# t0037799/INT8InferenceEngine

Measured on AMD Instinct MI355X. Metric: images/sec AlexNet-INT8 224x224 bs=1000, higher is better.
Workload: dtype int8; 1 GPU; alexnet INT8 forward + top-1, 3x224x224 input, global batch 1000 sharded over 1 GPU(s); global_batch=1000, per_gpu_batch=1000, parallelism=batch-shard x1 + logits all-gather

## Files before the change

int8inferenceengine_amd/csrc/i8ie_stem.hip:

```cpp
#include <cstdio>
#include <cstdlib>
#include <type_traits>
#include <vector>

#include "i8ie_stem.h"
#include "i8ie_stem_common.h"

#if !defined(STEM_DMA_VEC)
#define STEM_DMA_VEC 0
#endif

#if defined(STEM_PRIO_SWAP)
#define STEM_VPRIO 0
#define STEM_MPRIO 3
#endif

namespace {

__device__ __forceinline__ uint32_t quant_exact(float x, float scale, float zpf, float rscale) {
  const float est = __builtin_fmaf(x, rscale, zpf);
  const float fr = __builtin_amdgcn_fractf(est);
  if (__builtin_fabsf(est) < 1024.0f && __builtin_fabsf(fr - 0.5f) <= 0.5f - 9.765625e-4f)
    return (uint32_t)((int)est) & 0xFFu;
  const float t = x / scale + zpf;
  return (uint32_t)((int)t) & 0xFFu;
}

template <bool F32>
__global__ __launch_bounds__(256) void quantize_s2d_kernel(const void* __restrict__ xin, uint8_t* __restrict__ out, uint32_t total,
                                                           int c, int h, int w, int HY, int WX, int pad, float scale, float zpf,
                                                           float rscale, uint32_t zp) {
  const uint32_t gstride = gridDim.x * 256u;
  const size_t cs = (size_t)h * w;
  for (uint32_t e = blockIdx.x * 256u + threadIdx.x; e < total; e += gstride) {
    const uint32_t d = e & 3u, t0 = e >> 2;
    const uint32_t t1 = t0 / (uint32_t)WX, X = t0 - t1 * WX;
    const uint32_t img = t1 / (uint32_t)HY, Y = t1 - img * HY;
    const int y = (int)(4 * Y + d) - pad, x0 = (int)(4 * X) - pad;
    const bool yin = y >= 0 && y < h;
    const int yc = y < 0 ? 0 : (y >= h ? h - 1 : y);
    uint32_t q[12];
    if constexpr (F32) {
      const float* plane = static_cast<const float*>(xin) + ((size_t)img * c * h + yc) * w;
      const bool vec = (w & 1) == 0 && (pad & 1) == 0 && w >= 4 && (reinterpret_cast<uintptr_t>(xin) & 7u) == 0;
      const int xb = x0 < 0 ? 0 : (x0 > w - 4 ? w - 4 : x0);
      const int sft = x0 - xb;
#pragma unroll
      for (int ch = 0; ch < 3; ++ch) {
        const float* row = plane + (size_t)(ch < c ? ch : 0) * cs;
        float L[4];
        if (vec) {
          const float2 a = *reinterpret_cast<const float2*>(row + xb), b = *reinterpret_cast<const float2*>(row + xb + 2);
          L[0] = a.x; L[1] = a.y; L[2] = b.x; L[3] = b.y;
        } else {
#pragma unroll
          for (int i = 0; i < 4; ++i) {
            const int xx = xb + i;
            L[i] = row[xx < 0 ? 0 : (xx >= w ? w - 1 : xx)];
          }
        }
#pragma unroll
        for (int px = 0; px < 4; ++px) {
          int i = px + sft;
          i = i < 0 ? 0 : (i > 3 ? 3 : i);
          const float v = i == 0 ? L[0] : (i == 1 ? L[1] : (i == 2 ? L[2] : L[3]));
          q[px * 3 + ch] = quant_exact(v, scale, zpf, rscale);
        }
      }
    } else {
      const uint8_t* plane = static_cast<const uint8_t*>(xin) + ((size_t)img * c * h + yc) * w;
#pragma unroll
      for (int ch = 0; ch < 3; ++ch) {
        const uint8_t* row = plane + (size_t)(ch < c ? ch : 0) * cs;
#pragma unroll
        for (int px = 0; px < 4; ++px) {
          const int xx = x0 + px;
          q[px * 3 + ch] = row[xx < 0 ? 0 : (xx >= w ? w - 1 : xx)];
        }
      }
    }
    uint32_t wd[3] = {0, 0, 0};
#pragma unroll
    for (int px = 0; px < 4; ++px) {
      const int xx = x0 + px;
      const bool in = yin && xx >= 0 && xx < w;
#pragma unroll
      for (int ch = 0; ch < 3; ++ch) {
        const uint32_t v = (in && ch < c) ? q[px * 3 + ch] : zp;
        const int b = px * 3 + ch;
        wd[b >> 2] |= v << (8 * (b & 3));
      }
    }
    uint32_t* o = reinterpret_cast<uint32_t*>(out) + (size_t)e * 3;
    o[0] = wd[0] ^ 0x80808080u;
    o[1] = wd[1] ^ 0x80808080u;
    o[2] = wd[2] ^ 0x80808080u;
  }
}

template <int NG, int KS, bool ACC, bool PC>
__global__ __launch_bounds__(512, 2) void stem_conv_kernel(StemArgs p) {
  uint8_t* const smem = stem_smem;
  const int tid = threadIdx.x, lane = tid & 63;
  const int wave_hw = __builtin_amdgcn_readfirstlane(tid >> 6);
  const int wave = p.role_split ? ((wave_hw & 2) << 1) | ((wave_hw >> 2) << 1) | (wave_hw & 1) : wave_hw;
  const int hh = lane >> 5, l31 = lane & 31;

  const int n_units = p.n_img << p.lg_parts;
  const int n_mine = ((int)blockIdx.x < n_units) ? (n_units - 1 - (int)blockIdx.x) / (int)gridDim.x + 1 : 0;
  if (n_mine == 0) return;
  const int T = p.T, G = n_mine * T, RING = p.RING;
  const int pmask = p.parts - 1;

  for (int i = tid; i < p.N; i += 512) reinterpret_cast<int*>(smem + p.lds_ocp)[i] = p.ocp[i];
  for (int i = tid; i < KS * 64; i += 512) {
    const int j = i >> 6, ln = i & 63;
    *reinterpret_cast<v4i*>(smem + p.lds_bfrag + i * 16) =
        *reinterpret_cast<const v4i*>(p.B + (size_t)((NG - 1) * 32 + (ln & 31)) * p.Kpad + j * 32 + (ln >> 5) * 16);
  }
  stem_fill_tables(p, smem, tid, T, RING);
  __syncthreads();
  auto strip_fetch = [&](int unit, int t, v4i& a, v4i& b) {
    const int idx = (unit & pmask) * T + t;
    a = *reinterpret_cast<const v4i*>(smem + p.lds_tab + idx * 32);
    b = *reinterpret_cast<const v4i*>(smem + p.lds_tab + idx * 32 + 16);
  };
  auto strip_decode = [&](const v4i& a, const v4i& b) {
    StemStrip e;
    e.lo = __builtin_amdgcn_readfirstlane(a.x); e.hi = __builtin_amdgcn_readfirstlane(a.y);
    e.poff = __builtin_amdgcn_readfirstlane(a.z); e.pbytes = __builtin_amdgcn_readfirstlane(a.w);
    e.j0 = __builtin_amdgcn_readfirstlane(b.x); e.j1 = __builtin_amdgcn_readfirstlane(b.y);
    e.lom = __builtin_amdgcn_readfirstlane(b.z); e.jm = __builtin_amdgcn_readfirstlane(b.w);
    return e;
  };
  auto strip = [&](int unit, int t) {
    v4i a, b;
    strip_fetch(unit, t, a, b);
    return strip_decode(a, b);
  };
  auto adv_of = [&](int unit) { return __builtin_amdgcn_readfirstlane(reinterpret_cast<const int*>(smem + p.lds_adv)[unit & pmask]); };
  auto patch_dma = [&](int unit, const StemStrip& e, int pb) {
    if (e.pbytes <= 0) return;
    const __amdgpu_buffer_rsrc_t rs = __builtin_amdgcn_make_buffer_rsrc(
        const_cast<uint8_t*>(p.img + (size_t)(unit >> p.lg_parts) * p.img_pitch + (unsigned)e.poff), 0, e.pbytes, 0x00020000);
    const int pieces = (e.pbytes + 1023) >> 10;
    uint8_t* dst = smem + p.lds_patch + pb * p.patchB;
    for (int q = wave & 3; q < pieces; q += 4)
      __builtin_amdgcn_raw_ptr_buffer_load_lds(rs, (__attribute__((address_space(3))) void*)(dst + q * 1024), 16, (q * 64 + lane) * 16, 0, 0, 0);
  };

  if (wave < 4) {
#if defined(STEM_MPRIO)
    __builtin_amdgcn_s_setprio(STEM_MPRIO);
#endif
    constexpr int NA = NG - 1;
    v4i breg[NA > 0 ? NA : 1][KS];
#pragma unroll
    for (int g = 0; g < NA; ++g) {
      const int8_t* brow = p.B + (size_t)(g * 32 + l31) * p.Kpad + hh * 16;
#pragma unroll
      for (int j = 0; j < KS; ++j) breg[g][j] = *reinterpret_cast<const v4i*>(brow + j * 32);
    }
    int koff[KS];
    {
      int q = hh, run = 0, rem = hh;
#pragma unroll
      for (int j = 0; j < KS; ++j) {
        koff[j] = q < p.nch ? run * p.rowB + rem * 16 : 0;
        q += 2;
        rem += 2;
        while (rem >= p.RC) {
          rem -= p.RC;
          ++run;
        }
      }
    }
    const int pp = wave * 32 + l31;
    int lr = (int)((float)pp * p.rcpOW), lx = pp - lr * p.OW;
    if (lx < 0) { lx += p.OW; --lr; } else if (lx >= p.OW) { lx -= p.OW; ++lr; }
    const int aoff = (lr * p.sq * p.WX + lx * p.sq) * 48;
    const int roff = lx * p.pitchP + 16 * hh;
    int t = 0, un = (int)blockIdx.x, ib = 0, pbuf = 0;
    int tn = 0, imn = (int)blockIdx.x;
    auto next_n = [&]() {
      if (++tn == T) {
        tn = 0;
        imn += (int)gridDim.x;
      }
    };
    StemStrip e = strip(imn, tn);
    patch_dma(imn, e, 0);
    next_n();
    v4i fa, fb;
    strip_fetch(imn, tn, fa, fb);
    asm volatile("s_waitcnt vmcnt(0)" ::: "memory");
    STEM_BAR();
    for (int g = 0; g < G; ++g) {
      StemStrip en{};
      if (g + 1 < G) {
        en = strip_decode(fa, fb);
        if (!STEM_DMA_VEC) patch_dma(imn, en, pbuf ^ 1);
        next_n();
      }
      const int npx = (e.hi - e.lo) * p.OW;
      if (wave * 32 < npx) {
        const bool valid = pp < npx;
        const uint8_t* abase = smem + p.lds_patch + pbuf * p.patchB + (valid ? aoff : 0);
        int slot = ib + e.lom;
        if (slot >= RING) slot -= RING;
        int ls = slot + lr;
        if (ls >= RING) ls -= RING;
        uint8_t* const rbase = smem + p.lds_ring + ls * p.ringRowB + roff;
        v16i acc[NG];
        const v16i z = {0, 0, 0, 0, 0, 0, 0, 0, 0, 0, 0, 0, 0, 0, 0, 0};
        uint8_t* const wbase = valid ? rbase : smem + p.lds_dump + lane * 16;
        auto ring_store = [&](auto ggc, auto qc) {
          constexpr int gg = decltype(ggc)::value, q = decltype(qc)::value;
          v4i v;
          v.x = acc[gg][q * 4 + 0]; v.y = acc[gg][q * 4 + 1]; v.z = acc[gg][q * 4 + 2]; v.w = acc[gg][q * 4 + 3];
          *reinterpret_cast<v4i*>(wbase + (gg * 32 + 8 * q) * 4) = v;
        };
        {
          constexpr int DB = KS < 4 ? KS : 4;
          v4i ring[DB], bring[DB];
          const uint8_t* const bbase = smem + p.lds_bfrag + lane * 16;
          static_for<0, DB>([&](auto jc) {
            constexpr int j = decltype(jc)::value;
            ring[j] = *reinterpret_cast<const v4i*>(abase + koff[j]);
            bring[j] = *reinterpret_cast<const v4i*>(bbase + j * 1024);
          });
          __builtin_amdgcn_sched_barrier(0);
          static_for<0, KS>([&](auto jc) {
            constexpr int j = decltype(jc)::value;
            const v4i af = ring[j % DB], bf = bring[j % DB];
            if constexpr (j + DB < KS) {
              ring[j % DB] = *reinterpret_cast<const v4i*>(abase + koff[j + DB]);
              bring[j % DB] = *reinterpret_cast<const v4i*>(bbase + (j + DB) * 1024);
              __builtin_amdgcn_sched_barrier(0);
            }
#pragma unroll
            for (int gg = 0; gg < NA; ++gg) acc[gg] = __builtin_amdgcn_mfma_i32_32x32x32_i8(breg[gg][j], af, j == 0 ? z : acc[gg], 0, 0, 0);
            acc[NG - 1] = __builtin_amdgcn_mfma_i32_32x32x32_i8(bf, af, j == 0 ? z : acc[NG - 1], 0, 0, 0);
            __builtin_amdgcn_sched_barrier(0);
          });
          if constexpr (NA > 0)
            static_for<0, 4 * NA>([&](auto ic) { ring_store(std::integral_constant<int, decltype(ic)::value / 4>{}, std::integral_constant<int, decltype(ic)::value % 4>{}); });
        }
        static_for<0, 4>([&](auto qc) { ring_store(std::integral_constant<int, NG - 1>{}, qc); });
      }
      strip_fetch(imn, tn, fa, fb);
      if (!STEM_DMA_VEC) asm volatile("s_waitcnt vmcnt(0)" ::: "memory");
      STEM_BAR();
      if (++t == T) {
        t = 0;
        ib += adv_of(un);
        if (ib >= RING) ib -= RING;
        un += (int)gridDim.x;
      }
      pbuf ^= 1;
      e = en;
    }
    STEM_BAR();
    return;
  }

  const int vt = (wave - 4) * 64 + lane;
  const int vwave = wave - 4;
#if !defined(STEM_VPRIO)
#define STEM_VPRIO 0
#endif
  if (STEM_VPRIO) __builtin_amdgcn_s_setprio(STEM_VPRIO);
  const I8ieRequant rq = p.rq;
  const int lo_relu = p.relu_lo;
  const float lof = (float)lo_relu;
  const int N4 = p.N >> 2;
  const int PHp = p.PH + 2 * p.ob, PWp = p.PW + 2 * p.ob;
  const __amdgpu_buffer_rsrc_t rsO =
      __builtin_amdgcn_make_buffer_rsrc(p.out, 0, p.out_bytes, 0x00020000);
  const int hg = ((l31 >= 4 && l31 < 12) || (l31 >= 16 && l31 < 20) || l31 >= 28) ? 1 : 0;
  const int gi = hg == 0 ? (l31 < 4 ? l31 : (l31 < 16 ? l31 - 8 : l31 - 12)) : (l31 < 12 ? l31 - 4 : (l31 < 20 ? l31 - 8 : l31 - 16));
  const int pl = gi & 7;
  const int ql = 2 * (2 * hh + hg) + (gi >> 3);
  const int nqo = N4 >> 3, npo = (p.PW + 7) >> 3, ntask = nqo * npo;
  constexpr int PITCH = NG * 128 + 16;
  const int rd_lane = pl * p.ps * PITCH + ql * 16;
  const int st_lane = pl * p.N + ql * 4;

  constexpr int UN = 3;
  struct PoolTask {
    int rd, st, oc;
  };
  auto task_of = [&](int k) {
    int po = k < ntask ? k : 0, qo = 0;
    while (po >= npo) {
      po -= npo;
      ++qo;
    }
    const bool ok = 8 * po + pl < p.PW;
    PoolTask t;
    t.rd = (ok ? rd_lane : ql * 16) + (8 * po) * p.ps * PITCH + qo * 128;
    t.st = ok && k < ntask ? (8 * po) * p.N + qo * 32 + st_lane : (int)0x80000000;
    t.oc = p.lds_ocp + (qo * 8 + ql) * 16;
    return t;
  };
  PoolTask tk0[UN];
#pragma unroll
  for (int u = 0; u < UN; ++u) tk0[u] = task_of(vwave + 4 * u);
  v4i oc0[UN];
#pragma unroll
  for (int u = 0; u < UN; ++u) oc0[u] = *reinterpret_cast<const v4i*>(smem + tk0[u].oc);
  int nst = 0;
  auto pool_rows = [&](auto pkc, int im, int ib, const StemStrip& e) {
    constexpr int PK = decltype(pkc)::value;
    int rm = ib + e.jm;
    if (rm >= RING) rm -= RING;
    for (int j = e.j0; j < e.j1; ++j) {
      int rowoff[PK];
#pragma unroll
      for (int dy = 0; dy < PK; ++dy) {
        const int sl = rm + dy;
        rowoff[dy] = p.lds_ring + (sl >= RING ? sl - RING : sl) * p.ringRowB;
      }
      const int orow = ((im * PHp + j + p.ob) * PWp + p.ob) * p.N;
      auto round = [&](const PoolTask (&tk)[UN], const v4i (&ocv)[UN]) {
        float4 msq[UN];
        if constexpr (PC) {
#pragma unroll
          for (int u = 0; u < UN; ++u) msq[u] = *reinterpret_cast<const float4*>(p.msv + ((tk[u].oc - p.lds_ocp) >> 2));
        }
        v4i v[UN][PK * PK];
#pragma unroll
        for (int u = 0; u < UN; ++u)
#pragma unroll
          for (int dy = 0; dy < PK; ++dy) {
            const uint8_t* const a = smem + (rowoff[dy] + tk[u].rd);
#pragma unroll
            for (int dx = 0; dx < PK; ++dx) v[u][dy * PK + dx] = *reinterpret_cast<const v4i*>(a + dx * PITCH);
          }
        uint32_t d[UN];
        float worst[UN];
        int c4[UN][4];
#pragma unroll
        for (int u = 0; u < UN; ++u) {
          v4i m = v[u][0];
#pragma unroll
          for (int tt = 1; tt < PK * PK; ++tt) {
            m.x = m.x > v[u][tt].x ? m.x : v[u][tt].x;
            m.y = m.y > v[u][tt].y ? m.y : v[u][tt].y;
            m.z = m.z > v[u][tt].z ? m.z : v[u][tt].z;
            m.w = m.w > v[u][tt].w ? m.w : v[u][tt].w;
          }
          c4[u][0] = m.x + ocv[u].x; c4[u][1] = m.y + ocv[u].y;
          c4[u][2] = m.z + ocv[u].z; c4[u][3] = m.w + ocv[u].w;
          if constexpr (PC) d[u] = i8ie_requant_est4_pc(c4[u], rq, msq[u], lof, worst[u]);
          else d[u] = i8ie_requant_est4(c4[u], rq, lof, worst[u]);
        }
        float wmin = worst[0];
#pragma unroll
        for (int u = 1; u < UN; ++u) wmin = __builtin_fminf(wmin, worst[u]);
        if (!i8ie_requant_est_ok(wmin)) {
#pragma unroll
          for (int u = 0; u < UN; ++u)
            if (!i8ie_requant_est_ok(worst[u])) {
              if constexpr (PC) d[u] = i8ie_requant_exact4_pc(c4[u], rq, p.sbv + ((tk[u].oc - p.lds_ocp) >> 2), lo_relu);
              else d[u] = i8ie_requant_exact4(c4[u], rq, lo_relu);
            }
        }
#pragma unroll
        for (int u = 0; u < UN; ++u) __builtin_amdgcn_raw_buffer_store_b32(d[u] ^ p.xor_out, rsO, tk[u].st, orow, 0);
        nst += UN;
      };
      round(tk0, oc0);
      for (int k0 = vwave + 4 * UN; k0 < ntask; k0 += 4 * UN) {
        PoolTask tk[UN];
        v4i ocv[UN];
#pragma unroll
        for (int u = 0; u < UN; ++u) {
          tk[u] = task_of(k0 + 4 * u);
          ocv[u] = *reinterpret_cast<const v4i*>(smem + tk[u].oc);
        }
        round(tk, ocv);
      }
      rm += p.ps;
      if (rm >= RING) rm -= RING;
    }
  };
  auto dump_acc = [&](int im, int ib, const StemStrip& e) {
    const int tasks = (e.hi - e.lo) * p.OW * N4;
    const float rn4 = 1.0f / (float)N4;
    for (int id = vt; id < tasks; id += 256) {
      int t1 = (int)((float)id * rn4), qq = id - t1 * N4;
      if (qq < 0) { qq += N4; --t1; } else if (qq >= N4) { qq -= N4; ++t1; }
      int r = 0, x = t1;
      while (x >= p.OW) {
        x -= p.OW;
        ++r;
      }
      int sl = ib + e.lom + r;
      while (sl >= RING) sl -= RING;
      const v4i v = *reinterpret_cast<const v4i*>(smem + p.lds_ring + sl * p.ringRowB + x * p.pitchP + qq * 16);
      const v4i o = *reinterpret_cast<const v4i*>(smem + p.lds_ocp + qq * 16);
      const int4 c = make_int4(v.x + o.x, v.y + o.y, v.z + o.z, v.w + o.w);
      *reinterpret_cast<int4*>(p.acc + ((size_t)im * (size_t)(p.OH * p.OW) + (size_t)((e.lo + r) * p.OW + x)) * (size_t)p.N + qq * 4) = c;
    }
  };
  auto wait_vm_keep = [&](int keep) {
    switch (keep < 16 ? keep : 16) {
      case 0: asm volatile("s_waitcnt vmcnt(0)" ::: "memory"); break;
      case 1: asm volatile("s_waitcnt vmcnt(1)" ::: "memory"); break;
      case 2: asm volatile("s_waitcnt vmcnt(2)" ::: "memory"); break;
      case 3: asm volatile("s_waitcnt vmcnt(3)" ::: "memory"); break;
      case 4: asm volatile("s_waitcnt vmcnt(4)" ::: "memory"); break;
      case 5: asm volatile("s_waitcnt vmcnt(5)" ::: "memory"); break;
      case 6: asm volatile("s_waitcnt vmcnt(6)" ::: "memory"); break;
      case 7: asm volatile("s_waitcnt vmcnt(7)" ::: "memory"); break;
      case 8: asm volatile("s_waitcnt vmcnt(8)" ::: "memory"); break;
      case 9: asm volatile("s_waitcnt vmcnt(9)" ::: "memory"); break;
      case 10: asm volatile("s_waitcnt vmcnt(10)" ::: "memory"); break;
      case 11: asm volatile("s_waitcnt vmcnt(11)" ::: "memory"); break;
      case 12: asm volatile("s_waitcnt vmcnt(12)" ::: "memory"); break;
      case 13: asm volatile("s_waitcnt vmcnt(13)" ::: "memory"); break;
      case 14: asm volatile("s_waitcnt vmcnt(14)" ::: "memory"); break;
      case 15: asm volatile("s_waitcnt vmcnt(15)" ::: "memory"); break;
      default: asm volatile("s_waitcnt vmcnt(16)" ::: "memory"); break;
    }
  };

  int t1 = 0, im1 = (int)blockIdx.x, ib1 = 0;
  int tn = 1, imn = (int)blockIdx.x;
  if (tn == T) {
    tn = 0;
    imn += (int)gridDim.x;
  }
  v4i fa, fb;
  strip_fetch(im1, t1, fa, fb);
  STEM_BAR();
  for (int g = 0; g <= G; ++g) {
    if (STEM_DMA_VEC && g + 1 < G) {
      patch_dma(imn, strip(imn, tn), (g + 1) & 1);
      if (++tn == T) {
        tn = 0;
        imn += (int)gridDim.x;
      }
      nst = 0;
    }
    if (g >= 1) {
      const StemStrip e = strip_decode(fa, fb);
      const int img = im1 >> p.lg_parts;
      if (e.j1 > e.j0) {
        if (p.pk == 3) pool_rows(std::integral_constant<int, 3>{}, img, ib1, e);
        else if (p.pk == 2) pool_rows(std::integral_constant<int, 2>{}, img, ib1, e);
        else pool_rows(std::integral_constant<int, 1>{}, img, ib1, e);
      }
      if constexpr (ACC) {
        if (e.hi > e.lo) dump_acc(img, ib1, e);
      }
      if (++t1 == T) {
        t1 = 0;
        ib1 += adv_of(im1);
        if (ib1 >= RING) ib1 -= RING;
        im1 += (int)gridDim.x;
      }
    }
    strip_fetch(im1, t1, fa, fb);
    if constexpr (ACC) wait_vm_keep(0);
    else if (STEM_DMA_VEC) wait_vm_keep(nst);
    STEM_BAR();
  }
}

template <int NG, int KS, bool ACC, bool PC>
int launch_stem_t(i8ie_ctx* ctx, const StemArgs& a, int grid, int lds) {
  static bool raised[64] = {};
  const int dev = ctx->device & 63;
  if (!raised[dev]) {
    I8IE_HIP_TRY(hipFuncSetAttribute(reinterpret_cast<const void*>(&stem_conv_kernel<NG, KS, ACC, PC>), hipFuncAttributeMaxDynamicSharedMemorySize, 160 * 1024));
    raised[dev] = true;
  }
  stem_conv_kernel<NG, KS, ACC, PC><<<grid, 512, lds, ctx->stream>>>(a);
  I8IE_LAUNCH_CHECK();
  return I8IE_OK;
}
template <int NG, int KS>
int launch_stem(i8ie_ctx* ctx, const StemArgs& a, int grid, int lds) {
  if (a.msv != nullptr)
    return a.acc != nullptr ? launch_stem_t<NG, KS, true, true>(ctx, a, grid, lds) : launch_stem_t<NG, KS, false, true>(ctx, a, grid, lds);
  return a.acc != nullptr ? launch_stem_t<NG, KS, true, false>(ctx, a, grid, lds) : launch_stem_t<NG, KS, false, false>(ctx, a, grid, lds);
}

struct StemPlan {
  int KC4, KA4, HY, WX, K2, KS, KST, NR, first, T, parts, pk, ps, PH, PW, carry, RING, pitchP, ringRowB, patchB, lds_tab, lds_adv, lds_dump, lds_bfrag, lds;
};

bool stem_plan(int c, int stride, int N, int KH, int KW, int OH, int OW, int pool_k, int pool_s, int parts, StemPlan* out) {
  if (c > 3 || c < 1 || stride < 4 || stride % 4 != 0) return false;
  if (N % 32 != 0 || N < 32 || N > 96) return false;
  if (pool_k == 1 && pool_s > 1) return false;
  StemPlan s{};
  const int sq = stride / 4;
  s.KC4 = (KH + 3) / 4;
  s.KA4 = (KW + 3) / 4;
  s.HY = (OH - 1) * sq + s.KC4;
  s.WX = (OW - 1) * sq + s.KA4;
  s.K2 = s.KC4 * s.KA4 * 48;
  s.KS = (s.K2 + 31) / 32;
  if (s.KS > kStemMaxKS || s.KS < 2) return false;
  s.pk = pool_k > 1 ? pool_k : 1;
  s.ps = pool_k > 1 ? pool_s : 1;
  if (s.ps < 1 || s.ps > s.pk || s.pk > 3) return false;
  if (s.pk > OH || s.pk > OW) return false;
  s.PH = (OH - s.pk) / s.ps + 1;
  s.PW = (OW - s.pk) / s.ps + 1;
  s.carry = s.pk - s.ps;
  int NR = kStemPix / OW;
  NR -= NR % s.ps;
  if (NR < 1 || NR < s.carry) return false;
  if (NR > 8) NR = 8 - 8 % s.ps;
  s.NR = NR;
  s.first = s.carry > 0 ? s.carry : NR;
  if (s.first > OH) s.first = OH;
  if (parts != 1 && parts != 2 && parts != 4) return false;
  if (s.PH < 2 * parts) return false;
  s.parts = parts;
  auto J0_of = [&](int q) { return q * s.PH / parts; };
  auto R0_of = [&](int q) { return J0_of(q) * s.ps; };
  auto R1_of = [&](int q) { return q + 1 == parts ? OH : (J0_of(q + 1) - 1) * s.ps + s.pk; };
  s.T = 1;
  for (int q = 0; q < parts; ++q) {
    const int rows = R1_of(q) - R0_of(q);
    const int t = 1 + (rows > s.first ? (rows - s.first + NR - 1) / NR : 0);
    if (t > s.T) s.T = t;
  }
  s.RING = 2 * NR + s.carry;
  s.pitchP = N * 4 + 16;
  s.ringRowB = OW * s.pitchP;
  const int prmax = (NR - 1) * sq + s.KC4;
  s.patchB = ((prmax * s.WX * 48 + 1023) & ~1023) + 1024;
  if (s.T * parts > 256) return false;
  s.KST = s.KS <= 6 ? 6 : (s.KS <= 10 ? 10 : kStemMaxKS);
  s.lds_tab = 2 * s.patchB + s.RING * s.ringRowB + N * 4 + 64;
  s.lds_adv = s.lds_tab + s.T * parts * 32;
  s.lds_dump = s.lds_adv + 16;
  s.lds_bfrag = s.lds_dump + 2048;
  s.lds = s.lds_bfrag + s.KST * 1024;
  if (s.lds > 160 * 1024) return false;
  for (int qa = 0; qa < parts; ++qa)
    for (int qb = 0; qb < parts; ++qb) {
      const int q_of[2] = {qa, qb};
      const int base[2] = {0, R1_of(qa) - R0_of(qa)};
      auto hi_of = [&](int u, int t) { const int v = R0_of(q_of[u]) + s.first + t * s.NR; return v < R1_of(q_of[u]) ? v : R1_of(q_of[u]); };
      auto lo_of = [&](int u, int t) { return t == 0 ? R0_of(q_of[u]) : hi_of(u, t - 1); };
      auto done = [&](int u, int hi) {
        const int J0 = J0_of(q_of[u]), J1 = q_of[u] + 1 == parts ? s.PH : J0_of(q_of[u] + 1);
        if (hi < s.pk) return J0;
        int e = (hi - s.pk) / s.ps + 1;
        e = e < J1 ? e : J1;
        return e > J0 ? e : J0;
      };
      for (int g = 1; g < 2 * s.T; ++g) {
        const int u1 = (g - 1) / s.T, t1 = (g - 1) % s.T;
        const int j0 = t1 == 0 ? J0_of(q_of[u1]) : done(u1, lo_of(u1, t1)), j1 = done(u1, hi_of(u1, t1));
        if (j1 <= j0) continue;
        const int lo_read = base[u1] + j0 * s.ps - R0_of(q_of[u1]);
        const int u2 = g / s.T, t2 = g % s.T;
        const int wlo = base[u2] + lo_of(u2, t2) - R0_of(q_of[u2]), whi = base[u2] + hi_of(u2, t2) - 1 - R0_of(q_of[u2]);
        if (whi >= wlo && whi - lo_read + 1 > s.RING) return false;
      }
    }
  *out = s;
  return true;
}

}

int i8ie_stem_supported(int c, int stride, int N, int KH, int KW, int OH, int OW, int pool_k, int pool_s) {
  StemPlan s;
  return stem_plan(c, stride, N, KH, KW, OH, OW, pool_k, pool_s, 1, &s) ? 1 : 0;
}

int i8ie_stem_kpad(int KH, int KW) {
  const int KC4 = (KH + 3) / 4, KA4 = (KW + 3) / 4;
  const int ks = (KC4 * KA4 * 48 + 31) / 32;
  return (ks <= 6 ? 6 : ks <= 10 ? 10 : kStemMaxKS) * 32;
}
int i8ie_stem_kindex(int KW, int ch, int kh, int kw) {
  const int KA4 = (KW + 3) / 4;
  return (kh / 4) * (KA4 * 48) + (kw / 4) * 48 + (kh % 4) * 12 + (kw % 4) * 3 + ch;
}

size_t i8ie_stem_scratch_bytes(int n, int KH, int KW, int stride, int OH, int OW) {
  const int sq = stride / 4;
  const size_t HY = (size_t)(OH - 1) * sq + (KH + 3) / 4, WX = (size_t)(OW - 1) * sq + (KW + 3) / 4;
  return (size_t)n * HY * WX * 48;
}

int i8ie_stem_launch(i8ie_ctx* ctx, const I8ieStemCall& c) {
  static int cus[64] = {};
  const int dev = ctx->device & 63;
  if (cus[dev] == 0) {
    hipDeviceProp_t prop;
    I8IE_HIP_TRY(hipGetDeviceProperties(&prop, ctx->device));
    cus[dev] = prop.multiProcessorCount > 0 ? prop.multiProcessorCount : 256;
  }
  StemPlan s;
  int parts = 1;
  const int ncu = i8ie_cus(ctx, cus[dev]);
  while (parts < 4 && (long)c.n * parts * 4 < (long)ncu * 3) parts *= 2;
  if (ctx->pick.stem_whole) parts = 1;
  while (parts > 1 && !stem_plan(c.c, c.stride, c.N, c.KH, c.KW, c.OH, c.OW, c.pool_k, c.pool_s, parts, &s)) parts /= 2;
  if (!stem_plan(c.c, c.stride, c.N, c.KH, c.KW, c.OH, c.OW, c.pool_k, c.pool_s, parts, &s)) {
    i8ie_set_error("i8ie_stem_launch: geometry not supported");
    return I8IE_ERR_STATE;
  }
  const size_t img_pitch = (size_t)s.HY * s.WX * 48;
  const size_t out_bytes = (size_t)c.n * (s.PH + 2 * c.ob) * (s.PW + 2 * c.ob) * c.N;
  I8IE_REQUIRE(img_pitch < ((size_t)1 << 31) && out_bytes < ((size_t)1 << 31), "i8ie_stem_launch: tensor beyond the 32-bit offset range");
  I8IE_REQUIRE((size_t)c.n * 4 * s.HY * s.WX < ((size_t)1 << 32) - 65536, "i8ie_stem_launch: batch too large for one launch");
  {
    const uint32_t total = (uint32_t)((size_t)c.n * s.HY * s.WX * 4);
    I8ieProfScope prof(ctx, c.x != nullptr ? "quantize_s2d_f32" : "repack_s2d_u8", 0.0,
                       (c.x != nullptr ? 4.0 : 1.0) * c.n * c.c * c.h * c.w + (double)c.n * img_pitch);
    uint32_t blocks = (total + 255) / 256;
    if (blocks > 256 * 128) blocks = 256 * 128;
    const float rs = 1.0f / c.q_scale;
    if (c.x != nullptr)
      quantize_s2d_kernel<true><<<blocks, 256, 0, ctx->stream>>>(c.x, c.scratch, total, c.c, c.h, c.w, s.HY, s.WX, c.pad, c.q_scale,
                                                                (float)c.q_zp, rs, (uint32_t)(c.q_zp & 0xFF));
    else
      quantize_s2d_kernel<false><<<blocks, 256, 0, ctx->stream>>>(c.xu8, c.scratch, total, c.c, c.h, c.w, s.HY, s.WX, c.pad, 1.0f, 0.0f,
                                                                 1.0f, (uint32_t)(c.q_zp & 0xFF));
    I8IE_LAUNCH_CHECK();
  }
  StemArgs a{};
  a.img = c.scratch;
  a.img_pitch = (unsigned)img_pitch;
  a.n_img = c.n;
  a.WX = s.WX; a.rowB = s.WX * 48;
  a.OH = c.OH; a.OW = c.OW; a.sq = c.stride / 4; a.KC4 = s.KC4;
  a.NR = s.NR; a.first = s.first; a.T = s.T;
  a.pk = s.pk; a.ps = s.ps; a.PH = s.PH; a.PW = s.PW;
  a.B = c.B; a.Kpad = c.Kpad; a.N = c.N; a.ocp = c.ocp;
  a.rq = i8ie_make_requant(c.s_in, c.s_w, c.s_out, c.zp_out);
  a.relu_lo = c.relu ? c.zp_out : 0;
  a.out = c.out; a.ob = c.ob; a.xor_out = c.out_s8 ? 0x80808080u : 0u;
  a.acc = c.acc;
  a.msv = c.msv; a.sbv = c.sbv;
  a.pitchP = s.pitchP; a.ringRowB = s.ringRowB; a.RING = s.RING;
  a.patchB = s.patchB;
  a.lds_patch = 0;
  a.lds_ring = 2 * s.patchB;
  a.lds_ocp = a.lds_ring + s.RING * s.ringRowB;
  a.lds_tab = s.lds_tab;
  a.lds_dump = s.lds_dump;
  a.lds_bfrag = s.lds_bfrag;
  a.out_bytes = (unsigned)out_bytes;
  a.rcpOW = 1.0f / (float)c.OW;
  a.RC = s.KA4 * 3;
  a.nch = s.KC4 * a.RC;
  a.parts = s.parts;
  a.lg_parts = s.parts == 4 ? 2 : (s.parts == 2 ? 1 : 0);
  a.lds_adv = s.lds_adv;
  int grid = ncu;
  if (grid > c.n * s.parts) grid = c.n * s.parts;
  const double ops = 2.0 * c.n * c.OH * c.OW * (double)c.N * c.c * c.KH * c.KW;
  const double bytes = (double)c.n * img_pitch + (double)out_bytes;
  a.role_split = ctx->pick.stem_simd_roles ? 1 : 0;
  I8ieProfScope prof(ctx, s.pk > 1 ? "stem_conv_pool" : "stem_conv", ops, bytes);
  const int NG = c.N / 32;
#define I8IE_STEM_KS(NGV)                                                   \
  if (s.KS <= 6) return launch_stem<NGV, 6>(ctx, a, grid, s.lds);           \
  if (s.KS <= 10) return launch_stem<NGV, 10>(ctx, a, grid, s.lds);         \
  return launch_stem<NGV, kStemMaxKS>(ctx, a, grid, s.lds);
  if (NG == 1) { I8IE_STEM_KS(1) }
  if (NG == 2) { I8IE_STEM_KS(2) }
  I8IE_STEM_KS(3)
#undef I8IE_STEM_KS
}
```

Before: 782,900 images/sec.

## Reuse overlapping max-pool row maxima and streamline stem quantize/space-to-depth kernel

The pooling stage now folds each pool row horizontally once and carries the overlapping rows' horizontal maxima in registers to the next output row, so it reads only the new stride rows from LDS instead of all PK*PK windows. The quantize/space-to-depth kernel replaces the per-element divisions with one block-level index decomposition plus a short carry loop. It also checks all 12 quantization estimates together before falling back to the exact path, and packs the bytes with perm instructions. The risks are extra register pressure from the carried row state and a correctness dependency on the `fresh` reset. That reset only fires for the first task batch of each strip; later batches on the same row re-read everything.

```diff
diff --git a/int8inferenceengine_amd/csrc/i8ie_stem.hip b/int8inferenceengine_amd/csrc/i8ie_stem.hip
--- a/int8inferenceengine_amd/csrc/i8ie_stem.hip
+++ b/int8inferenceengine_amd/csrc/i8ie_stem.hip
@@ -13,6 +13,10 @@
 #if defined(STEM_PRIO_SWAP)
 #define STEM_VPRIO 0
 #define STEM_MPRIO 3
+#endif
+
+#if !defined(STEM_QBLOCKS)
+#define STEM_QBLOCKS (256 * 128)
 #endif
 
 namespace {
@@ -30,42 +34,61 @@
 __global__ __launch_bounds__(256) void quantize_s2d_kernel(const void* __restrict__ xin, uint8_t* __restrict__ out, uint32_t total,
                                                            int c, int h, int w, int HY, int WX, int pad, float scale, float zpf,
                                                            float rscale, uint32_t zp) {
-  const uint32_t gstride = gridDim.x * 256u;
+  const uint32_t gstride = gridDim.x * 256u, W4 = 4u * (uint32_t)WX;
   const size_t cs = (size_t)h * w;
-  for (uint32_t e = blockIdx.x * 256u + threadIdx.x; e < total; e += gstride) {
-    const uint32_t d = e & 3u, t0 = e >> 2;
-    const uint32_t t1 = t0 / (uint32_t)WX, X = t0 - t1 * WX;
-    const uint32_t img = t1 / (uint32_t)HY, Y = t1 - img * HY;
-    const int y = (int)(4 * Y + d) - pad, x0 = (int)(4 * X) - pad;
+  for (uint32_t e0 = blockIdx.x * 256u; e0 < total; e0 += gstride) {
+    const uint32_t r0 = e0 / W4, img0 = r0 / (uint32_t)HY;
+    uint32_t off = e0 - r0 * W4 + threadIdx.x, Y = r0 - img0 * (uint32_t)HY, img = img0;
+    while (off >= W4) {
+      off -= W4;
+      if (++Y == (uint32_t)HY) {
+        Y = 0;
+        ++img;
+      }
+    }
+    const uint32_t e = e0 + threadIdx.x;
+    if (e >= total) continue;
+    const int y = (int)(4 * Y + (off & 3u)) - pad, x0 = (int)(off & ~3u) - pad;
     const bool yin = y >= 0 && y < h;
     const int yc = y < 0 ? 0 : (y >= h ? h - 1 : y);
     uint32_t q[12];
     if constexpr (F32) {
       const float* plane = static_cast<const float*>(xin) + ((size_t)img * c * h + yc) * w;
       const bool vec = (w & 1) == 0 && (pad & 1) == 0 && w >= 4 && (reinterpret_cast<uintptr_t>(xin) & 7u) == 0;
-      const int xb = x0 < 0 ? 0 : (x0 > w - 4 ? w - 4 : x0);
-      const int sft = x0 - xb;
+      int xo[4];
+      if (vec) {
+        xo[0] = x0 < 0 ? 0 : (x0 > w - 2 ? w - 2 : x0);
+        xo[2] = x0 + 2 < 0 ? 0 : (x0 > w - 4 ? w - 2 : x0 + 2);
+      } else {
+#pragma unroll
+        for (int i = 0; i < 4; ++i) xo[i] = x0 + i < 0 ? 0 : (x0 + i >= w ? w - 1 : x0 + i);
+      }
+      float v[12];
 #pragma unroll
       for (int ch = 0; ch < 3; ++ch) {
         const float* row = plane + (size_t)(ch < c ? ch : 0) * cs;
-        float L[4];
         if (vec) {
-          const float2 a = *reinterpret_cast<const float2*>(row + xb), b = *reinterpret_cast<const float2*>(row + xb + 2);
-          L[0] = a.x; L[1] = a.y; L[2] = b.x; L[3] = b.y;
+          const float2 a = *reinterpret_cast<const float2*>(row + xo[0]), b = *reinterpret_cast<const float2*>(row + xo[2]);
+          v[ch] = a.x; v[3 + ch] = a.y; v[6 + ch] = b.x; v[9 + ch] = b.y;
         } else {
 #pragma unroll
-          for (int i = 0; i < 4; ++i) {
-            const int xx = xb + i;
-            L[i] = row[xx < 0 ? 0 : (xx >= w ? w - 1 : xx)];
-          }
-        }
-#pragma unroll
-        for (int px = 0; px < 4; ++px) {
-          int i = px + sft;
-          i = i < 0 ? 0 : (i > 3 ? 3 : i);
-          const float v = i == 0 ? L[0] : (i == 1 ? L[1] : (i == 2 ? L[2] : L[3]));
-          q[px * 3 + ch] = quant_exact(v, scale, zpf, rscale);
-        }
+          for (int px = 0; px < 4; ++px) v[px * 3 + ch] = row[xo[px]];
+        }
+      }
+      float est[12];
+      bool ok = true;
+#pragma unroll
+      for (int i = 0; i < 12; ++i) {
+        est[i] = __builtin_fmaf(v[i], rscale, zpf);
+        const float fr = __builtin_amdgcn_fractf(est[i]);
+        ok = ok && __builtin_fabsf(est[i]) < 1024.0f && __builtin_fabsf(fr - 0.5f) <= 0.5f - 9.765625e-4f;
+      }
+      if (ok) {
+#pragma unroll
+        for (int i = 0; i < 12; ++i) q[i] = (uint32_t)((int)est[i]);
+      } else {
+#pragma unroll
+        for (int i = 0; i < 12; ++i) q[i] = quant_exact(v[i], scale, zpf, rscale);
       }
     } else {
       const uint8_t* plane = static_cast<const uint8_t*>(xin) + ((size_t)img * c * h + yc) * w;
@@ -79,22 +102,21 @@
         }
       }
     }
-    uint32_t wd[3] = {0, 0, 0};
 #pragma unroll
     for (int px = 0; px < 4; ++px) {
       const int xx = x0 + px;
       const bool in = yin && xx >= 0 && xx < w;
 #pragma unroll
-      for (int ch = 0; ch < 3; ++ch) {
-        const uint32_t v = (in && ch < c) ? q[px * 3 + ch] : zp;
-        const int b = px * 3 + ch;
-        wd[b >> 2] |= v << (8 * (b & 3));
-      }
+      for (int ch = 0; ch < 3; ++ch)
+        if (!(in && ch < c)) q[px * 3 + ch] = zp;
     }
     uint32_t* o = reinterpret_cast<uint32_t*>(out) + (size_t)e * 3;
-    o[0] = wd[0] ^ 0x80808080u;
-    o[1] = wd[1] ^ 0x80808080u;
-    o[2] = wd[2] ^ 0x80808080u;
+#pragma unroll
+    for (int k = 0; k < 3; ++k) {
+      const uint32_t lo = __builtin_amdgcn_perm(q[4 * k + 1], q[4 * k], 0x0c0c0400u);
+      const uint32_t hi = __builtin_amdgcn_perm(q[4 * k + 3], q[4 * k + 2], 0x0c0c0400u);
+      o[k] = __builtin_amdgcn_perm(hi, lo, 0x05040100u) ^ 0x80808080u;
+    }
   }
 }
 
@@ -310,8 +332,11 @@
 #pragma unroll
   for (int u = 0; u < UN; ++u) oc0[u] = *reinterpret_cast<const v4i*>(smem + tk0[u].oc);
   int nst = 0;
-  auto pool_rows = [&](auto pkc, int im, int ib, const StemStrip& e) {
-    constexpr int PK = decltype(pkc)::value;
+  v4i hc[UN][2];
+  bool fresh = true;
+  auto max3 = [](int a, int b, int c) { const int m = a > b ? a : b; return m > c ? m : c; };
+  auto pool_rows = [&](auto pkc, auto psc, int im, int ib, const StemStrip& e) {
+    constexpr int PK = decltype(pkc)::value, PS = decltype(psc)::value, CR = PK - PS;
     int rm = ib + e.jm;
     if (rm >= RING) rm -= RING;
     for (int j = e.j0; j < e.j1; ++j) {
@@ -322,34 +347,73 @@
         rowoff[dy] = p.lds_ring + (sl >= RING ? sl - RING : sl) * p.ringRowB;
       }
       const int orow = ((im * PHp + j + p.ob) * PWp + p.ob) * p.N;
-      auto round = [&](const PoolTask (&tk)[UN], const v4i (&ocv)[UN]) {
+      auto round = [&](const PoolTask (&tk)[UN], const v4i (&ocv)[UN], v4i (&hcr)[UN][2], const bool whole) {
         float4 msq[UN];
         if constexpr (PC) {
 #pragma unroll
           for (int u = 0; u < UN; ++u) msq[u] = *reinterpret_cast<const float4*>(p.msv + ((tk[u].oc - p.lds_ocp) >> 2));
         }
-        v4i v[UN][PK * PK];
+        auto read_row = [&](v4i (&r)[PK], int u, int dy) {
+          const uint8_t* const a = smem + (rowoff[dy] + tk[u].rd);
+#pragma unroll
+          for (int dx = 0; dx < PK; ++dx) r[dx] = *reinterpret_cast<const v4i*>(a + dx * PITCH);
+        };
+        auto fold_row = [&](const v4i (&r)[PK]) {
+          v4i m;
+          if constexpr (PK == 1) {
+            m = r[0];
+          } else if constexpr (PK == 2) {
+            m.x = r[0].x > r[1].x ? r[0].x : r[1].x; m.y = r[0].y > r[1].y ? r[0].y : r[1].y;
+            m.z = r[0].z > r[1].z ? r[0].z : r[1].z; m.w = r[0].w > r[1].w ? r[0].w : r[1].w;
+          } else {
+            m.x = max3(r[0].x, r[1].x, r[2].x); m.y = max3(r[0].y, r[1].y, r[2].y);
+            m.z = max3(r[0].z, r[1].z, r[2].z); m.w = max3(r[0].w, r[1].w, r[2].w);
+          }
+          return m;
+        };
+        v4i top[UN][CR > 0 ? CR : 1][PK], v[UN][PS][PK];
+        if constexpr (CR > 0) {
+          if (whole) {
+#pragma unroll
+            for (int u = 0; u < UN; ++u)
+#pragma unroll
+              for (int dy = 0; dy < CR; ++dy) read_row(top[u][dy], u, dy);
+          }
+        }
 #pragma unroll
         for (int u = 0; u < UN; ++u)
 #pragma unroll
-          for (int dy = 0; dy < PK; ++dy) {
-            const uint8_t* const a = smem + (rowoff[dy] + tk[u].rd);
-#pragma unroll
-            for (int dx = 0; dx < PK; ++dx) v[u][dy * PK + dx] = *reinterpret_cast<const v4i*>(a + dx * PITCH);
+          for (int dy = 0; dy < PS; ++dy) read_row(v[u][dy], u, CR + dy);
+        if constexpr (CR > 0) {
+          if (whole) {
+#pragma unroll
+            for (int u = 0; u < UN; ++u)
+#pragma unroll
+              for (int dy = 0; dy < CR; ++dy) hcr[u][dy] = fold_row(top[u][dy]);
           }
+        }
         uint32_t d[UN];
         float worst[UN];
         int c4[UN][4];
 #pragma unroll
         for (int u = 0; u < UN; ++u) {
-          v4i m = v[u][0];
-#pragma unroll
-          for (int tt = 1; tt < PK * PK; ++tt) {
-            m.x = m.x > v[u][tt].x ? m.x : v[u][tt].x;
-            m.y = m.y > v[u][tt].y ? m.y : v[u][tt].y;
-            m.z = m.z > v[u][tt].z ? m.z : v[u][tt].z;
-            m.w = m.w > v[u][tt].w ? m.w : v[u][tt].w;
+          v4i hm[PK];
+#pragma unroll
+          for (int dy = 0; dy < CR; ++dy) hm[dy] = hcr[u][dy];
+#pragma unroll
+          for (int dy = 0; dy < PS; ++dy) hm[CR + dy] = fold_row(v[u][dy]);
+          v4i m;
+          if constexpr (PK == 1) {
+            m = hm[0];
+          } else if constexpr (PK == 2) {
+            m.x = hm[0].x > hm[1].x ? hm[0].x : hm[1].x; m.y = hm[0].y > hm[1].y ? hm[0].y : hm[1].y;
+            m.z = hm[0].z > hm[1].z ? hm[0].z : hm[1].z; m.w = hm[0].w > hm[1].w ? hm[0].w : hm[1].w;
+          } else {
+            m.x = max3(hm[0].x, hm[1].x, hm[2].x); m.y = max3(hm[0].y, hm[1].y, hm[2].y);
+            m.z = max3(hm[0].z, hm[1].z, hm[2].z); m.w = max3(hm[0].w, hm[1].w, hm[2].w);
           }
+#pragma unroll
+          for (int dy = 0; dy < CR; ++dy) hcr[u][dy] = hm[PS + dy];
           c4[u][0] = m.x + ocv[u].x; c4[u][1] = m.y + ocv[u].y;
           c4[u][2] = m.z + ocv[u].z; c4[u][3] = m.w + ocv[u].w;
           if constexpr (PC) d[u] = i8ie_requant_est4_pc(c4[u], rq, msq[u], lof, worst[u]);
@@ -370,16 +434,17 @@
         for (int u = 0; u < UN; ++u) __builtin_amdgcn_raw_buffer_store_b32(d[u] ^ p.xor_out, rsO, tk[u].st, orow, 0);
         nst += UN;
       };
-      round(tk0, oc0);
+      round(tk0, oc0, hc, fresh);
+      fresh = false;
       for (int k0 = vwave + 4 * UN; k0 < ntask; k0 += 4 * UN) {
         PoolTask tk[UN];
-        v4i ocv[UN];
+        v4i ocv[UN], hx[UN][2];
 #pragma unroll
         for (int u = 0; u < UN; ++u) {
           tk[u] = task_of(k0 + 4 * u);
           ocv[u] = *reinterpret_cast<const v4i*>(smem + tk[u].oc);
         }
-        round(tk, ocv);
+        round(tk, ocv, hx, true);
       }
       rm += p.ps;
       if (rm >= RING) rm -= RING;
@@ -448,15 +513,25 @@
       const StemStrip e = strip_decode(fa, fb);
       const int img = im1 >> p.lg_parts;
       if (e.j1 > e.j0) {
-        if (p.pk == 3) pool_rows(std::integral_constant<int, 3>{}, img, ib1, e);
-        else if (p.pk == 2) pool_rows(std::integral_constant<int, 2>{}, img, ib1, e);
-        else pool_rows(std::integral_constant<int, 1>{}, img, ib1, e);
+        auto pool = [&](auto pkc, auto psc) { pool_rows(pkc, psc, img, ib1, e); };
+        using std::integral_constant;
+        if (p.pk == 3) {
+          if (p.ps == 2) pool(integral_constant<int, 3>{}, integral_constant<int, 2>{});
+          else if (p.ps == 1) pool(integral_constant<int, 3>{}, integral_constant<int, 1>{});
+          else pool(integral_constant<int, 3>{}, integral_constant<int, 3>{});
+        } else if (p.pk == 2) {
+          if (p.ps == 2) pool(integral_constant<int, 2>{}, integral_constant<int, 2>{});
+          else pool(integral_constant<int, 2>{}, integral_constant<int, 1>{});
+        } else {
+          pool(integral_constant<int, 1>{}, integral_constant<int, 1>{});
+        }
       }
       if constexpr (ACC) {
         if (e.hi > e.lo) dump_acc(img, ib1, e);
       }
       if (++t1 == T) {
         t1 = 0;
+        fresh = true;
         ib1 += adv_of(im1);
         if (ib1 >= RING) ib1 -= RING;
         im1 += (int)gridDim.x;
@@ -621,7 +696,7 @@
     I8ieProfScope prof(ctx, c.x != nullptr ? "quantize_s2d_f32" : "repack_s2d_u8", 0.0,
                        (c.x != nullptr ? 4.0 : 1.0) * c.n * c.c * c.h * c.w + (double)c.n * img_pitch);
     uint32_t blocks = (total + 255) / 256;
-    if (blocks > 256 * 128) blocks = 256 * 128;
+    if (blocks > STEM_QBLOCKS) blocks = STEM_QBLOCKS;
     const float rs = 1.0f / c.q_scale;
     if (c.x != nullptr)
       quantize_s2d_kernel<true><<<blocks, 256, 0, ctx->stream>>>(c.x, c.scratch, total, c.c, c.h, c.w, s.HY, s.WX, c.pad, c.q_scale,
```

New measurement: 765,900 images/sec. -2.2%, worse.
